# patrikhuber/superviseddescent

Hardware: AMD Instinct MI355X
Metric: faces/sec RCR-22 detect (batch 4096) (higher is better)
Workload: dtype f32; 1 GPU; RCR-22 detect, batch 4096 synthetic 256x256 u8 faces per GPU, 4 cascade levels (UoCTTI HOG 5x5 cells, cell 11/10/8/6, 4 orientations, F=8801, M=44), model trained on-GPU on 100000 synthetic faces (shipped .bin absent from the reference checkout); batch_per_gpu=4096, levels=4

## Files before the change

### superviseddescent_amd/csrc/sdm_apply.hip

```cpp
#include "sdm_kernels.h"
#include <stdlib.h>

#pragma clang fp contract(off)
#include "sdm_ied.h"

namespace {

typedef float f32x4 __attribute__((ext_vector_type(4)));

#define APPLY_WAVES 4

template <int RT, int NT>
__global__ void __launch_bounds__(APPLY_WAVES * 64)
apply_partial_kernel(const float* __restrict__ feat, long long ldf, int N, int kgroups,
                     const float* __restrict__ Rt, long long ldr, float* __restrict__ partial, int splits)
{
    __shared__ float red[APPLY_WAVES - 1][RT * NT][4][64];
    const int lane = threadIdx.x & 63, wave = threadIdx.x >> 6;
    const int li = lane & 15, lq = lane >> 4;
    const int row0 = blockIdx.x * (16 * RT);
    const int split = blockIdx.y;
    const int g0 = (int)(((long long)kgroups * split) / splits);
    const int g1 = (int)(((long long)kgroups * (split + 1)) / splits);

// ... 265 lines not shown
    for (int o = 32; o; o >>= 1) v = __builtin_fmaxf(v, __shfl_xor(v, o));
    if ((threadIdx.x & 63) == 0) part[threadIdx.x >> 6] = v;
    __syncthreads();
    if (threadIdx.x == 0) out[blockIdx.x] = __builtin_bit_cast(unsigned, __builtin_fmaxf(__builtin_fmaxf(part[0], part[1]), __builtin_fmaxf(part[2], part[3])));
}

__global__ void __launch_bounds__(256) apply_planes_kernel(const float* __restrict__ Rt, long long ldr, int Mp, int KG, af16x8* __restrict__ planes,
                                                           const unsigned* __restrict__ rmax)
{
    const long long u = (long long)blockIdx.x * 256 + threadIdx.x;
    if (u >= (long long)KG * Mp) return;
    const int kg = (int)(u / Mp), col = (int)(u % Mp);
    const float scale = __builtin_ldexpf(1.0f, 14 - apply_f16_exponent(rmax[col]));
    const float* src = Rt + (long long)col * ldr + 8 * kg;
    af16x8 p1, p2;
#pragma unroll
    for (int j = 0; j < 8; ++j) {
        const float v = src[j] * scale;
        const _Float16 h1 = (_Float16)v;
        p1[j] = h1; p2[j] = (_Float16)(v - (float)h1);
    }
    planes[u] = p1; planes[(size_t)KG * Mp + u] = p2;
}

__global__ void apply_reduce_kernel(const float* __restrict__ partial, int splits, int N, int Mp, int M,
                                    const float* __restrict__ x_in, float* __restrict__ x_out, int L,
                                    EyeIdxDev eyes)
{
    const long long t = (long long)blockIdx.x * blockDim.x + threadIdx.x;
    if (t >= (long long)N * M) return;
    const int row = (int)(t / M), col = (int)(t - (long long)row * M);
    const float* xr = x_in + (long long)row * M;
    const float xc = xr[col];
    float scale = 1.0f;
    if (eyes.nre > 0) {
        const float n = (float)(1.0 / device_ied_rows(xr, L, eyes));
        scale = 1.0f / n;
    }
    float u = 0.0f;
    const float* pp = partial + (long long)row * Mp + col;
    const long long sstride = (long long)N * Mp;
    constexpr int RB = 24;
    for (int s0 = 0; s0 < splits; s0 += RB) {
        float v[RB];
#pragma unroll
        for (int j = 0; j < RB; ++j) v[j] = pp[(long long)(s0 + j < splits ? s0 + j : splits - 1) * sstride];
#pragma unroll
        for (int j = 0; j < RB; ++j) u = s0 + j < splits ? u + v[j] : u;
    }
    x_out[t] = xc - u * scale;
}

__global__ void targets_kernel(const float* __restrict__ x, const float* __restrict__ xstar, int N, int L,
                               EyeIdxDev eyes, float* __restrict__ feat, long long ldf, int bcol0)
{
    const int M = 2 * L;
    const long long t = (long long)blockIdx.x * blockDim.x + threadIdx.x;
    if (t >= (long long)N * M) return;
    const int row = (int)(t / M), col = (int)(t - (long long)row * M);
    const float* xr = x + (long long)row * M;
    float n = 1.0f;
    if (eyes.nre > 0) n = (float)(1.0 / device_ied_rows(xr, L, eyes));
    feat[(long long)row * ldf + bcol0 + col] = (xr[col] - xstar[t]) * n;
}

__global__ void pack_regressor_kernel(const float* __restrict__ Rsol, int F, int M, int Mp, float* __restrict__ Rt,
                                      long long ldf, float* __restrict__ Rc)
{
    const long long t = (long long)blockIdx.x * blockDim.x + threadIdx.x;
    if (t >= (long long)Mp * ldf) return;
    const int j = (int)(t / ldf);
    const long long k = t - (long long)j * ldf;
    const float v = (k < F && j < M) ? Rsol[k * Mp + j] : 0.0f;
    Rt[t] = v;
    if (Rc && k < F && j < M) Rc[k * M + j] = v;
}

__global__ void subtract_templates_kernel(float* __restrict__ feat, long long ldf, const float* __restrict__ tmpl, int N, int F)
{
    const long long t = (long long)blockIdx.x * blockDim.x + threadIdx.x;
    if (t >= (long long)N * F) return;
    const int row = (int)(t / F), col = (int)(t - (long long)row * F);
    feat[(long long)row * ldf + col] -= tmpl[t];
// ... 251 lines not shown
```

### superviseddescent_amd/csrc/sdm_capi_context.hip

```cpp
#include "sdm_capi_internal.h"

extern "C" {

const char* sdm_last_error(void) { return err_string().c_str(); }

int sdm_device_count(void)
{
    int n = 0;
    if (hipGetDeviceCount(&n) != hipSuccess) return 0;
    return n;
}

sdm_ctx* sdm_create(int device)
{
    int n = 0;
    if (hipGetDeviceCount(&n) != hipSuccess || n <= 0) {
        fail(SDM_ERR_NO_DEVICE, "no HIP device available: this engine has no CPU fallback");
        return nullptr;
    }
    if (device < 0 || device >= n) { fail(SDM_ERR_INVALID, "device index out of range"); return nullptr; }
    hipDeviceProp_t prop;
    if (hipGetDeviceProperties(&prop, device) != hipSuccess) { fail(SDM_ERR_HIP, "hipGetDeviceProperties failed"); return nullptr; }
    if (strncmp(prop.gcnArchName, "gfx950", 6) != 0) {
        fail(SDM_ERR_NO_DEVICE, std::string("device is ") + prop.gcnArchName + ", kernels are built for gfx950 only");
// ... 7 lines not shown
    }
    c->own_stream = true;
    int prio_least = 0, prio_greatest = 0;
    (void)hipDeviceGetStreamPriorityRange(&prio_least, &prio_greatest);
    if (hipStreamCreateWithPriority(&c->solve_aux.stream, hipStreamNonBlocking, prio_least) != hipSuccess ||
        hipEventCreateWithFlags(&c->solve_aux.chain_done, hipEventDisableTiming) != hipSuccess ||
        hipEventCreateWithFlags(&c->solve_aux.tail_done, hipEventDisableTiming) != hipSuccess) {
        fail(SDM_ERR_HIP, "hipStreamCreate failed"); delete c; return nullptr;
    }
    if (c->status.ensure(1, true, c->stream) || c->lambda_dev.ensure(1, true, c->stream)) { delete c; return nullptr; }
    for (int b = 0; b < sdm_ctx::XBLOCKS_MAX; ++b)
        if (hipEventCreateWithFlags(&c->gram_ev[b], hipEventDisableTiming) != hipSuccess) { fail(SDM_ERR_HIP, "hipEventCreate failed"); delete c; return nullptr; }
    if (hipEventCreateWithFlags(&c->gram_xdone, hipEventDisableTiming) != hipSuccess) { fail(SDM_ERR_HIP, "hipEventCreate failed"); delete c; return nullptr; }
    return c;
}

void sdm_destroy(sdm_ctx* c)
{
    if (!c) return;
    hipError_t e = hipSetDevice(c->device); (void)e;
    e = hipStreamSynchronize(c->stream);
    if (c->solve_aux.stream) {
        e = hipStreamSynchronize(c->solve_aux.stream);
        e = hipEventDestroy(c->solve_aux.chain_done); e = hipEventDestroy(c->solve_aux.tail_done);
        for (int b = 0; b < sdm_ctx::XBLOCKS_MAX; ++b) if (c->gram_ev[b]) e = hipEventDestroy(c->gram_ev[b]);
        if (c->gram_xdone) e = hipEventDestroy(c->gram_xdone);
        e = hipStreamDestroy(c->solve_aux.stream);
    }
    drain_timing(c);
    for (auto ev : c->pool) { e = hipEventDestroy(ev); }
    c->img_owned.release(); c->img_off.release(); c->img_w.release(); c->img_h.release();
    c->img_stride.release(); c->img_idx.release(); c->x[0].release(); c->x[1].release();
    c->xstar.release(); c->tmpl.release(); c->feat.release(); c->patch_idx.release(); c->status.release();
    c->partial.release(); c->shard_stage.release(); c->G.release(); c->gpack.release(); c->fro.release(); c->Rsol.release(); c->winv.release(); c->gram_planes.release(); c->gram_flag.release(); c->upd_planes.release(); c->upd_maxdiag.release(); c->lambda_dev.release();
    for (auto& r : c->Rp) r.release();
    for (auto& r : c->Rd) r.release();
    c->cells.release(); c->qr_work.release();
    c->Rmax.release();
    c->pose.release();
    c->track.release();
    c->align.release();
    c->sweep.release();
    c->frames.release();
    c->upright.release();
    c->warp.release();
    for (auto& r : c->Rt) r.release();
    for (auto& q : c->plans) { q.lane_tab.release(); q.wb.release(); q.wb16.release(); q.pass_info.release(); q.cut.release(); q.taps.release(); q.pair_taps.release(); }
    if (c->own_stream) e = hipStreamDestroy(c->stream);
    delete c;
}

int sdm_set_stream(sdm_ctx* c, void* hip_stream)
{
    if (!c) return fail(SDM_ERR_INVALID, "null context");
    HIP_TRY(hipStreamSynchronize(c->stream));
    if (c->own_stream) { HIP_TRY(hipStreamDestroy(c->stream)); c->own_stream = false; }
    c->stream = (hipStream_t)hip_stream;
    return SDM_OK;
}

int sdm_synchronize(sdm_ctx* c)
{
    if (!c) return fail(SDM_ERR_INVALID, "null context");
    HIP_TRY(hipStreamSynchronize(c->stream));
    drain_timing(c);
    return SDM_OK;
}
// ... 393 lines not shown
```

### superviseddescent_amd/csrc/sdm_capi_debug.hip

```cpp
#include "sdm_capi_internal.h"

extern "C" {

int sdm_gram_device_ptr(sdm_ctx* c, void** p, size_t* count)
{
    if (!c || c->g_level < 0) return fail(SDM_ERR_INVALID, "no Gram matrix");
    *p = c->G.p; *count = (size_t)c->g_fp * c->g_ncols;
    return SDM_OK;
}

int sdm_x_device_ptr(sdm_ctx* c, void** p, size_t* count)
{
    if (!c || c->N <= 0) return fail(SDM_ERR_INVALID, "no x");
    *p = c->x[c->cur].p; *count = (size_t)c->N * c->M;
    return SDM_OK;
}

int sdm_features_device_ptr(sdm_ctx* c, void** p, long long* ld, int* n_rows)
{
    if (!c || c->feat_level < 0) return fail(SDM_ERR_INVALID, "no features");
    *p = c->feat.p; *ld = c->ldf; *n_rows = c->N;
    c->feat_bounded = false;
    return SDM_OK;
}
// ... 172 lines not shown
    if (!c) return fail(SDM_ERR_INVALID, "null context");
    c->fuse_apply = fused != 0;
    c->fuse_wide = fused == 2;
    c->split_store = split_store != 0;
    return SDM_OK;
}

int sdm_debug_gradient_table(sdm_ctx* c, int level, float* g, int* bin)
{
    if (!c || level < 0 || level >= (int)c->levels.size() || !g || !bin) return fail(SDM_ERR_INVALID, "bad arguments");
    HIP_TRY(hipSetDevice(c->device));
    const size_t n = 511 * 511;
    ScopedBuf<float> d_g; ScopedBuf<int> d_b;
    int rc;
    if ((rc = d_g.ensure(n)) || (rc = d_b.ensure(n))) return rc;
    sdm_launch_gradient_table(c->levels[level], d_g.p, d_b.p, c->stream);
    HIP_TRY(hipGetLastError());
    HIP_TRY(hipMemcpyAsync(g, d_g.p, n * sizeof(float), hipMemcpyDeviceToHost, c->stream));
    HIP_TRY(hipMemcpyAsync(bin, d_b.p, n * sizeof(int), hipMemcpyDeviceToHost, c->stream));
    HIP_TRY(hipStreamSynchronize(c->stream));
    d_g.release(); d_b.release();
    return SDM_OK;
}

int sdm_debug_set_option(sdm_ctx* c, const char* name, int value)
{
    if (!c || !name) return fail(SDM_ERR_INVALID, "bad arguments");
    const std::string n(name);
    if (n == "hog_no_pack") c->packing = value == 0;
    else if (n == "hog_two_load") c->hog_two_load = value != 0;
    else if (n == "hog_split_store") c->split_store = value != 0;
    else if (n == "detect_unfused") c->fuse_apply = value == 0;
    else if (n == "detect_fuse_wide") c->env_fuse_wide = value != 0;
    else if (n == "apply_f32") c->env_apply_f32 = value != 0;
    else if (n == "gram_f32") c->env_gram_f32 = value != 0;
    else if (n == "gram_bf16x3") c->env_gram_bf16 = value != 0;
    else if (n == "update_f32") c->solve_aux.upd_f32_only = value != 0 ? 1 : 0;
    else if (n == "gram_xblocks") c->env_xblocks = value;
    else if (n == "solve_upd_min_tiles") c->solve_aux.upd_min_tiles = value;
    else if (n == "solve_fine_head") c->solve_aux.fine_head_max = value;
    else if (n == "solve_bs_cap") c->solve_aux.bs_cap = value;
    else if (n == "solve_shard_emulate") c->env_shard_emulate = value;
    else return fail(SDM_ERR_INVALID, "sdm_debug_set_option: unknown option " + n);
    return SDM_OK;
}

int sdm_debug_update_f16(sdm_ctx* c, const float* P_host, int rows, int wcols, int wcols_factor, float factor_bound, float* C_host)
{
    if (!c || !P_host || !C_host || rows <= 0 || rows > 512 || rows % 128 || wcols <= 0 || wcols % 128 || wcols_factor <= 0 || wcols_factor > wcols || wcols_factor % 128)
        return fail(SDM_ERR_INVALID, "bad arguments");
    HIP_TRY(hipSetDevice(c->device));
    ScopedBuf<float> dP, dC; ScopedBuf<unsigned char> planes; ScopedBuf<unsigned> scales; ScopedBuf<int> status;
    int rc;
    if ((rc = dP.ensure((size_t)rows * wcols)) || (rc = dC.ensure((size_t)wcols * wcols)) || (rc = planes.ensure(sdm_update_f16_plane_bytes(512, wcols))) ||
        (rc = scales.ensure(4)) || (rc = status.ensure(1, true, c->stream)))
        return rc;
    HIP_TRY(hipMemcpyAsync(dP.p, P_host, (size_t)rows * wcols * sizeof(float), hipMemcpyHostToDevice, c->stream));
    HIP_TRY(hipMemcpyAsync(dC.p, C_host, (size_t)wcols * wcols * sizeof(float), hipMemcpyHostToDevice, c->stream));
    const unsigned sc[4] = {__builtin_bit_cast(unsigned, factor_bound), 0u, 0u, __builtin_bit_cast(unsigned, factor_bound)};
    HIP_TRY(hipMemcpyAsync(scales.p, sc, sizeof(sc), hipMemcpyHostToDevice, c->stream));
    sdm_launch_update_split_f16(dP.p, wcols, rows, wcols, wcols_factor, planes.p, scales.p, 0, status.p, c->stream, false);
    sdm_launch_update_f16(planes.p, rows, wcols, wcols_factor, dC.p, wcols, scales.p, 0, 0, 1 << 30, 0, 1, c->stream, 0);
    HIP_TRY(hipGetLastError());
    int st = 0;
    HIP_TRY(hipMemcpyAsync(&st, status.p, sizeof(int), hipMemcpyDeviceToHost, c->stream));
    HIP_TRY(hipMemcpyAsync(C_host, dC.p, (size_t)wcols * wcols * sizeof(float), hipMemcpyDeviceToHost, c->stream));
// ... 7 lines not shown
```

### superviseddescent_amd/csrc/sdm_capi_detect.hip

```cpp
#include "sdm_capi_internal.h"

namespace sdm_capi {

void fill_row_tab(HogLevelDev& lv)
{
    for (int d = 0; d < 64 && d < lv.S; ++d) {
        const HogRowConst rc = packed_row_const(d, lv.cell, lv.C);
        lv.row_tab[d][0] = rc.ws0;
        lv.row_tab[d][1] = rc.ws1;
        memcpy(&lv.row_tab[d][2], &rc.band, sizeof(int));
        lv.row_tab[d][3] = rc.w2;
    }
}



void drain_timing(sdm_ctx* c)
{
    for (auto& p : c->pending) {
        hipError_t e = hipEventSynchronize(p.b); (void)e;
        float ms = 0.f;
        if (hipEventElapsedTime(&ms, p.a, p.b) == hipSuccess) { c->t_ms[p.slot] += ms; c->t_n[p.slot] += 1; }
        if (!p.a_shared) c->pool.push_back(p.a);
        c->pool.push_back(p.b);
// ... 157 lines not shown
{
    if (c->feat_level != level) return fail(SDM_ERR_INVALID, "sdm_apply: features of this level not extracted");
    if (!c->have_R[level]) return fail(SDM_ERR_INVALID, "sdm_apply: no regressor set for this level");
    const int F = level_F(c, level);
    const int splits = sdm_apply_splits(c->N, F, c->M);
    int rc = c->partial.ensure((size_t)splits * c->N * Mp_of(c->M));
    if (rc) return rc;
    {
        Timer t(c, SDM_T_APPLY);
        sdm_launch_apply(c->feat.p, c->ldf, c->N, F, c->Rt[level].p, c->ldf, c->M, c->x[c->cur].p,
                         c->x[c->cur ^ 1].p, c->L, c->eyes, c->partial.p, splits, c->stream,
                         (c->feat_bounded && !c->env_apply_f32) ? c->Rp[level].p : nullptr,
                         (c->feat_bounded && !c->env_apply_f32 && c->Rp[level].p) ? c->Rmax.p + (size_t)level * Mp_of(c->M) : nullptr);
    }
    HIP_TRY(hipGetLastError());
    c->cur ^= 1;
    return SDM_OK;
}

bool fused_ok(const sdm_ctx* c, int level)
{
    return c->fuse_apply && (Mp_of(c->M) <= 64 || c->env_fuse_wide || c->fuse_wide) && split_ok(c, level) && c->have_R[level] && c->Rd[level].p &&
           c->Rp[level].p && c->tmpl_N == 0;
}
int detect_level_fused(sdm_ctx* c, int l)
{
    { const int rci = hog_checks(c, l); if (rci) return rci; }
    const int Mp = Mp_of(c->M);
    int rc;
    size_t cells_max = 0;
    for (size_t q = 0; q < c->levels.size(); ++q) { const size_t n = sdm_cells_floats(c->levels[q], c->N, c->L); if (n > cells_max) cells_max = n; }
    if ((rc = c->cells.ensure(cells_max)) || (rc = c->partial.ensure((size_t)c->L * c->N * Mp))) return rc;
    const HogLevelDev& lv = c->levels[l];
    {
        Timer t(c, SDM_T_HOG);
        sdm_launch_hog_cells(image_set(c), sample_index(c), c->x[c->cur].p, c->N, c->L, c->eyes, lv,
                             cells_plan(c, l), c->cells.p, c->patch_idx.p, c->status.p, c->stream);
    }
    {
        Timer t(c, SDM_T_APPLY);
        sdm_launch_desc_apply(lv, c->cells.p, c->plans[l].cut.p, c->N, c->L, c->M, c->Rd[l].p, c->Rmax.p + (size_t)l * Mp,
                              c->Rt[l].p, c->ldf, c->partial.p, c->stream);
        sdm_launch_apply_reduce(c->partial.p, c->L, c->N, c->M, c->x[c->cur].p, c->x[c->cur ^ 1].p, c->L, c->eyes, c->stream);
    }
    HIP_TRY(hipGetLastError());
    c->cur ^= 1;
    c->feat_level = -1;
    c->have_patch_idx = true;
    return SDM_OK;
}

int detect_level(sdm_ctx* c, int l)
{
    if (fused_ok(c, l)) return detect_level_fused(c, l);
    int rc = do_hog(c, l);
    if (!rc) rc = do_apply(c, l);
    return rc;
}

}

extern "C" {

int sdm_hog_features(sdm_ctx* c, int level, float* feat_host)
{
    if (!c || level < 0 || level >= (int)c->levels.size()) return fail(SDM_ERR_INVALID, "bad level");
    HIP_TRY(hipSetDevice(c->device));
    int rc = do_hog(c, level);
    if (rc) return rc;
    if (feat_host) {
        const int F = level_F(c, level);
        HIP_TRY(hipMemcpy2DAsync(feat_host, (size_t)F * sizeof(float), c->feat.p, (size_t)c->ldf * sizeof(float),
                                 (size_t)F * sizeof(float), c->N, hipMemcpyDeviceToHost, c->stream));
        HIP_TRY(hipStreamSynchronize(c->stream));
        return check_status(c);
    }
// ... 70 lines not shown
```

### superviseddescent_amd/csrc/sdm_capi_internal.h

```cpp
#pragma once
#include "../../include/sdm.h"
#include "sdm_kernels.h"

#include <dlfcn.h>
#include <limits.h>
#include <math.h>
#include <stdio.h>
#include <stdlib.h>
#include <string.h>
#include <string>
#include <vector>

namespace sdm_capi {


inline std::string& err_string() { static thread_local std::string e; return e; }

inline int fail(int code, const std::string& msg)
{
    err_string() = msg;
    return code;
}

constexpr long long SDM_FUSED_MAX_STRIDE = 1ll << 20;
// ... 77 lines not shown
    bool env_gram_f32 = false;
    bool env_gram_bf16 = false;
    int env_shard_emulate = 0;
    int hog_mode = SDM_HOG_COLUMNS;
    int Fmax = 0;
    long long ldf = 0;
    int rhs_tiles = 1;

    DevBuf<uint8_t> img_owned;
    const uint8_t* img_base = nullptr;
    DevBuf<long long> img_off;
    DevBuf<int> img_w, img_h, img_stride;
    int n_images = 0;
    bool narrow_images = false;
    DevBuf<int> img_idx;
    bool idx_identity = true;
    int n_idx = 0, max_idx = -1;

    int N = 0;
    DevBuf<float> x[2];
    int cur = 0;
    DevBuf<float> xstar;
    DevBuf<float> tmpl;
    int tmpl_F = 0, tmpl_N = 0;
    bool have_targets = false;
    DevBuf<float> feat;
    int feat_level = -1;
    int feat_wide_F = 0, feat_wide_N = 0;
    bool feat_bounded = false;
    DevBuf<int> patch_idx;
    bool have_patch_idx = false;
    DevBuf<int> status;
    DevBuf<float> partial;

    std::vector<DevBuf<float>> Rt;
    std::vector<DevBuf<unsigned char>> Rp;
    std::vector<DevBuf<unsigned char>> Rd;
    DevBuf<unsigned> Rmax;
    std::vector<bool> have_R;

    DevBuf<float> G;
    DevBuf<float> gpack;
    int g_ncols = 0;
    int g_fp = 0;
    int g_level = -1;
    DevBuf<double> fro;
    DevBuf<float> Rsol;
    DevBuf<float> winv;
    DevBuf<int> gram_flag;
    static const int XBLOCKS_MAX = 8;
    hipEvent_t gram_ev[XBLOCKS_MAX] = {}; hipEvent_t gram_xdone = nullptr;
    int gram_blocks = 0;
    int gram_block_c[XBLOCKS_MAX + 1] = {};
    int env_xblocks = -1;
    int gram_fallbacks = 0;
    int update_range_fallbacks = 0;
    int gram_f32_fallbacks = 0;
    DevBuf<unsigned char> gram_planes;
    DevBuf<float> lambda_dev;

    sdm_allreduce_fn allreduce = nullptr;
    void* allreduce_user = nullptr;
    int world_size = 1;
    void* rccl_comm = nullptr;
    int (*rccl_allreduce)(const void*, void*, size_t, int, int, void*, hipStream_t) = nullptr;
    int shard_rank = 0, shard_world = 0;
// ... 214 lines not shown
```

### superviseddescent_amd/csrc/sdm_desc.hip

```cpp
#include "sdm_kernels.h"
#include <stdlib.h>

#pragma clang fp contract(off)

namespace {

typedef float f32x4 __attribute__((ext_vector_type(4)));
typedef _Float16 f16x8 __attribute__((ext_vector_type(8)));
typedef unsigned u32x4 __attribute__((ext_vector_type(4)));

#define DS_WAVES 8
#ifndef DS_MINW
#define DS_MINW 6
#endif
#ifndef DS_ABL
#define DS_ABL 0
#endif

__host__ __device__ constexpr int desc_dim(int O, int variant) { return variant == 1 ? 3 * O + 4 : 4 * O; }
__host__ __device__ constexpr int desc_dp(int D) { return (D + 7) / 8 * 8; }
__host__ __device__ constexpr int desc_pk(int CC, int D) { return CC * desc_dp(D); }
__host__ __device__ constexpr int desc_kp(int P) { return (P + 31) / 32 * 32; }
__host__ __device__ constexpr int desc_ks(int P) { return ((P + 7) / 8) * 8 + 8; }
__host__ __device__ constexpr size_t desc_stage_bytes(int P, int FB) { return (size_t)2 * FB * desc_ks(P) * 2 + 64; }

__device__ inline int desc_f16_exponent(unsigned maxbits)
{
    const float b = __builtin_bit_cast(float, maxbits);
    if (!(b > 0.0f) || !(b < 3.0e38f)) return 14;
    return (int)((maxbits >> 23) & 0xff) - 127;
}

__host__ __device__ constexpr int desc_kparts(int PK) { return desc_kp(PK) / 32 <= 14 ? 2 : 4; }
__host__ __device__ constexpr int desc_nw(int PK, int W) { return W / desc_kparts(PK); }

template <int TO, int TC, int VARIANT, bool FUSED, int FB, int W = DS_WAVES, bool ONE = false>
__global__ void __launch_bounds__(W * 64, (TO > 4 && !FUSED) ? 2 : ((TO <= 4 && FUSED) ? DS_MINW : 4))
desc_kernel(const float* __restrict__ cells, const int* __restrict__ cut, int N, int L,
            float* __restrict__ feat, long long ldf, int has_bias,
            const u32x4* __restrict__ planes, int NT, const unsigned* __restrict__ rmax, const float* __restrict__ Rt, long long ldr,
            float* __restrict__ partial)
{
    constexpr int O = TO, C = TC, CC = C * C, D = desc_dim(TO, VARIANT), P = CC * D;
    constexpr int DP = desc_dp(D), PK = desc_pk(CC, D);
    constexpr int KP = desc_kp(PK), KS = desc_ks(PK), KSTEPS = KP / 32, MT = FB / 16;
    static_assert(CC <= 32, "one cell per lane, two patches per wave");
    extern __shared__ __attribute__((aligned(16))) unsigned char smem[];
    unsigned short* stage_hi = (unsigned short*)smem;
    unsigned short* stage_lo = stage_hi + (size_t)FB * KS;
    const int lane = threadIdx.x & 63, wave = threadIdx.x >> 6;
    const int tile = blockIdx.x / L, l = blockIdx.x - tile * L;
    const int half = lane >> 5, cell = lane & 31;
    const bool active = cell < CC;
    const int cc = active ? cell : CC - 1;
    const int x = cc / C, y = cc - x * C, ct = x * C + y, ci = y * C + x;
    const int xm = x > 0 ? x - 1 : 0, xp = x < C - 1 ? x + 1 : C - 1, ym = y > 0 ? y - 1 : 0, yp = y < C - 1 ? y + 1 : C - 1;
    const int lb = half * 32;
    const int iA = (lb + xm * C + ym) * 4, iB = (lb + x * C + ym) * 4, iC = (lb + xp * C + ym) * 4;
    const int iD = (lb + xm * C + y) * 4, iF = (lb + xp * C + y) * 4;
    const int iG = (lb + xm * C + yp) * 4, iH = (lb + x * C + yp) * 4, iI = (lb + xp * C + yp) * 4;
    const unsigned ipk0 = iA | iB << 8 | iC << 16 | iD << 24, ipk1 = iF | iG << 8 | iH << 16 | iI << 24;
    const int cutw = cut[l];
    const bool is_cut = (cutw & 1) != 0;
    const bool ld0 = x <= ((cutw >> 8) & 0xff), ld1 = x >= ((cutw >> 16) & 0xff);

    if (FUSED) {
        constexpr int PADW = KS - PK;
        for (int i = threadIdx.x; i < 2 * FB * PADW; i += W * 64) {
            const int piece = i / (FB * PADW), r = i - piece * (FB * PADW);
            const int m = r / PADW, k = PK + (r - m * PADW);
            (piece ? stage_lo : stage_hi)[(size_t)m * KS + k] = 0;
        }
        if (threadIdx.x < 32) ((unsigned short*)smem)[(size_t)2 * FB * KS + threadIdx.x] = 0;
    }

// ... 210 lines not shown
        }
    }
    }
    __syncthreads();
    float* red = (float*)smem;
    if (kp > 0) {
#pragma unroll
        for (int ti = 0; ti < MAXT; ++ti) {
            const int nt = ntl + ti * NW;
            if (nt >= NT) continue;
#pragma unroll
            for (int mt = 0; mt < MT; ++mt)
#pragma unroll
                for (int e = 0; e < 4; ++e) red[((((size_t)(kp - 1) * NT + nt) * MT + mt) * 4 + e) * 64 + lane_p] = acc[ti][mt][e];
        }
    }
    __syncthreads();
    if (kp == 0) {
#pragma unroll
        for (int ti = 0; ti < MAXT; ++ti) {
            const int nt = ntl + ti * NW;
            if (nt >= NT) continue;
            const int col = 16 * nt + li;
            const float unscale = __builtin_ldexpf(1.0f, -12 + (desc_f16_exponent(rmx[ti]) - 14));
            const float bias = biasv[ti];
#pragma unroll
            for (int mt = 0; mt < MT; ++mt)
#pragma unroll
                for (int e = 0; e < 4; ++e) {
                    float v = acc[ti][mt][e];
#pragma unroll
                    for (int q = 1; q < KPARTS; ++q) v += red[((((size_t)(q - 1) * NT + nt) * MT + mt) * 4 + e) * 64 + lane_p];
                    const int face = tile * FB + 16 * mt + 4 * lq + e;
                    if (face < N) partial[((long long)l * N + face) * Mp + col] = v * unscale + bias;
                }
        }
    }
}

__global__ void __launch_bounds__(256) desc_planes_kernel(const float* __restrict__ Rt, long long ldr, int L, int P, int C, int D, int DP, int KSTEPS, int NT,
                                                          const unsigned* __restrict__ rmax, f16x8* __restrict__ planes)
{
    const long long u = (long long)blockIdx.x * 256 + threadIdx.x;
    if (u >= (long long)L * KSTEPS * NT * 64) return;
    const int lane = (int)(u & 63);
    const long long frag = u >> 6;
    const int nt = (int)(frag % NT), ks = (int)((frag / NT) % KSTEPS), l = (int)(frag / ((long long)NT * KSTEPS));
    const int col = 16 * nt + (lane & 15), k0 = 32 * ks + 8 * (lane >> 4);
    const float scale = __builtin_ldexpf(1.0f, 14 - desc_f16_exponent(rmax[col]));
    const float* src = Rt + (long long)col * ldr + (long long)l * P;
    const int CC = C * C;
    f16x8 p1, p2;
#pragma unroll
    for (int j = 0; j < 8; ++j) {
        const int kk = k0 + j, cell = kk / DP, f = kk - cell * DP;
        const int y = cell / C, x = cell - y * C, ct = x * C + y;
        const float v = (cell < CC && f < D) ? src[f * CC + ct] * scale : 0.0f;
        const _Float16 h1 = (_Float16)v;
        p1[j] = h1; p2[j] = (_Float16)(v - (float)h1);
    }
    planes[frag * 128 + lane] = p1;
    planes[frag * 128 + 64 + lane] = p2;
}

template <int TO, int VARIANT, bool FUSED, int FB, int W = DS_WAVES, bool ONE = false>
void launch_desc(const float* cells, const int* cut, int N, int L, float* feat, long long ldf, int has_bias, const void* planes, int NT,
                 const unsigned* rmax, const float* Rt, long long ldr, float* partial, hipStream_t stream)
{
    const size_t lds = FUSED ? desc_stage_bytes(desc_pk(25, desc_dim(TO, VARIANT)), FB) + (FB == 16 ? 40 * 1024 : 0) : 0;
    const unsigned grid = (unsigned)(((long long)N + FB - 1) / FB * L);
    static unsigned long long seen = 0;
    if (FUSED && sdm_first_use_on_device(seen))
        SDM_SET_ATTR((const void*)desc_kernel<TO, 5, VARIANT, FUSED, FB, W, ONE>, hipFuncAttributeMaxDynamicSharedMemorySize, 160 * 1024);
    hipLaunchKernelGGL((desc_kernel<TO, 5, VARIANT, FUSED, FB, W, ONE>), dim3(grid), dim3(W * 64), lds, stream, cells, cut, N, L, feat, ldf,
                       has_bias, (const u32x4*)planes, NT, rmax, Rt, ldr, partial);
}

}

bool sdm_desc_supported(const HogLevelDev& lv) { return lv.C == 5 && (lv.O == 4 || lv.O == 9) && (lv.variant == 0 || lv.variant == 1); }

size_t sdm_cells_floats(const HogLevelDev& lv, int N, int L) { return (size_t)N * L * 2 * 2 * lv.O * lv.C * lv.C + 4; }

void sdm_launch_desc_store(const HogLevelDev& lv, const float* cells, const int* cut, int N, int L, float* feat, long long ldf, hipStream_t stream)
{
    if (N <= 0) return;
    const int hb = lv.fixed_h == 0 ? 1 : 0;
#define DS(O, V) launch_desc<O, V, false, 64>(cells, cut, N, L, feat, ldf, hb, nullptr, 0, nullptr, nullptr, 0, nullptr, stream)
    if (lv.O == 4) { if (lv.variant == 1) DS(4, 1); else DS(4, 0); }
    else { if (lv.variant == 1) DS(9, 1); else DS(9, 0); }
#undef DS
}

size_t sdm_desc_planes_bytes(const HogLevelDev& lv, int L, int M)
{
    const int KSTEPS = desc_kp(desc_pk(lv.C * lv.C, desc_dim(lv.O, lv.variant))) / 32, NT = (M + 15) / 16;
    return ((size_t)L * KSTEPS + 1) * NT * 2 * 64 * 16;
}

void sdm_launch_desc_planes(const HogLevelDev& lv, const float* Rt, long long ldr, int L, int M, const unsigned* rmax, void* planes, hipStream_t stream)
{
    const int D = desc_dim(lv.O, lv.variant), DP = desc_dp(D);
    const int KSTEPS = desc_kp(desc_pk(lv.C * lv.C, D)) / 32, NT = (M + 15) / 16;
    const long long total = (long long)L * KSTEPS * NT * 64;
    hipLaunchKernelGGL(desc_planes_kernel, dim3((unsigned)((total + 255) / 256)), dim3(256), 0, stream, Rt, ldr, L, lv.P, lv.C, D, DP, KSTEPS, NT, rmax, (f16x8*)planes);
    hipError_t e = hipMemsetAsync((unsigned char*)planes + (size_t)L * KSTEPS * NT * 2 * 64 * 16, 0, (size_t)NT * 2 * 64 * 16, stream); (void)e;
}

void sdm_launch_desc_apply(const HogLevelDev& lv, const float* cells, const int* cut, int N, int L, int M, const void* planes,
                           const unsigned* rmax, const float* Rt, long long ldr, float* partial, hipStream_t stream)
{
    if (N <= 0) return;
    const int hb = lv.fixed_h == 0 ? 1 : 0, NT = (M + 15) / 16;
#define DA(O, V, FB) do { \
        if (NT <= desc_nw(desc_pk(25, desc_dim(O, V)), DS_WAVES)) launch_desc<O, V, true, FB, DS_WAVES, true>(cells, cut, N, L, nullptr, 0, hb, planes, NT, rmax, Rt, ldr, partial, stream); \
        else launch_desc<O, V, true, FB>(cells, cut, N, L, nullptr, 0, hb, planes, NT, rmax, Rt, ldr, partial, stream); \
    } while (0)
    if (lv.O == 4) { if (lv.variant == 1) DA(4, 1, 32); else DA(4, 0, 32); }
    else { if (lv.variant == 1) DA(9, 1, 16); else DA(9, 0, 16); }
#undef DA
}
```

### superviseddescent_amd/csrc/sdm_ied.h

```cpp
#pragma once
#include "sdm_kernels.h"

__device__ inline double device_ied_rows(const float* __restrict__ xr, int L, const EyeIdxDev& e)
{
    float rx = 0.0f, ry = 0.0f, lx = 0.0f, ly = 0.0f;
    float vrx[SDM_MAX_EYE], vry[SDM_MAX_EYE], vlx[SDM_MAX_EYE], vly[SDM_MAX_EYE];
#pragma unroll
    for (int i = 0; i < SDM_MAX_EYE; ++i) {
        const int ir = e.re[i < e.nre ? i : 0], il = e.le[i < e.nle ? i : 0];
        vrx[i] = xr[ir]; vry[i] = xr[ir + L]; vlx[i] = xr[il]; vly[i] = xr[il + L];
    }
#pragma unroll
    for (int i = 0; i < SDM_MAX_EYE; ++i) {
        if (i < e.nre) { rx += vrx[i]; ry += vry[i]; }
        if (i < e.nle) { lx += vlx[i]; ly += vly[i]; }
    }
    rx /= (float)e.nre; ry /= (float)e.nre;
    lx /= (float)e.nle; ly /= (float)e.nle;
    float dxf = rx - lx, dyf = ry - ly;
    double dx = dxf, dy = dyf;
    return sqrt(dx * dx + dy * dy);
}
```

### superviseddescent_amd/csrc/sdm_kernels.h

```cpp
#pragma once
#include <hip/hip_runtime.h>
#include <cstdio>
#include <stdint.h>
#include "sdm_align_tensor_device.h"

#define SDM_SCALE_TAB 128
#define SDM_MAX_ORIENT 16
#define SDM_MAX_EYE 4

struct HogLevelDev {
    int variant;
    int C;
    int cell;
    int O;
    int S;
    int D;
    int P;
    float rel;
    int fixed_h;
    float ox[SDM_MAX_ORIENT];
    float oy[SDM_MAX_ORIENT];
    int n_sector;
    float sector_t[SDM_MAX_ORIENT / 2];
    alignas(16) float row_tab[64][4];
// ... 62 lines not shown
template <int CELL, int C>
struct HogRowConstTable {
    HogRowConst r[C * CELL] = {};
    constexpr HogRowConstTable() { for (int d = 0; d < C * CELL; ++d) r[d] = packed_row_const(d, CELL, C); }
};
const HogRowConst* sdm_hog_compiled_row_consts(int cell, int C);
#ifdef __cplusplus
#include <vector>
struct HogPlanHost {
    int G = 0, P = 0, n_main = 0, Gt = 0, Pt = 0, hist_slots = 2;
    std::vector<unsigned> lane_tab;
    std::vector<float> wb;
    std::vector<unsigned short> wb16;
    std::vector<int> pass_info;
    std::vector<int> cut;
};
bool sdm_hog_plan_build(const HogLevelDev& lv, int L, HogPlanHost& out);
#endif
void sdm_launch_hog_packed(const ImageSetDev& imgs, const int* img_idx, const float* x, int N, int L,
                           const EyeIdxDev& eyes, const HogLevelDev& lv, const HogPlanDev& plan, float* feat, long long ldf,
                           int* idx_out, int* status, hipStream_t stream);

void sdm_launch_hog_cells(const ImageSetDev& imgs, const int* img_idx, const float* x, int N, int L,
                          const EyeIdxDev& eyes, const HogLevelDev& lv, const HogPlanDev& plan, float* cells,
                          int* idx_out, int* status, hipStream_t stream);
bool sdm_hog_cells_row_carry(const HogLevelDev& lv, const HogPlanDev& plan);
bool sdm_hog_cells_pair_carry(const HogLevelDev& lv, const HogPlanDev& plan);

bool sdm_desc_supported(const HogLevelDev& lv);
size_t sdm_cells_floats(const HogLevelDev& lv, int N, int L);
void sdm_launch_desc_store(const HogLevelDev& lv, const float* cells, const int* cut, int N, int L, float* feat, long long ldf, hipStream_t stream);
size_t sdm_desc_planes_bytes(const HogLevelDev& lv, int L, int M);
void sdm_launch_desc_planes(const HogLevelDev& lv, const float* Rt, long long ldr, int L, int M, const unsigned* rmax, void* planes, hipStream_t stream);
void sdm_launch_desc_apply(const HogLevelDev& lv, const float* cells, const int* cut, int N, int L, int M, const void* planes,
                           const unsigned* rmax, const float* Rt, long long ldr, float* partial, hipStream_t stream);
void sdm_launch_apply_reduce(const float* partial, int splits, int N, int M, const float* x_in, float* x_out, int L,
                             const EyeIdxDev& eyes, hipStream_t stream);

size_t sdm_colpiv_qr_work_floats(int F);
bool sdm_colpiv_qr_supported(int F);
void sdm_launch_colpiv_qr_solve(float* G, long long ldg, int F, int rhs0, int nrhs, float* R_out, long long ldr, int r_rows,
                                float* work, int** rank_dev_out, hipStream_t stream);

void sdm_launch_hog_fast_profile(const ImageSetDev& imgs, const int* img_idx, const float* x, int N, int L,
                                 const EyeIdxDev& eyes, const HogLevelDev& lv, float* feat, long long ldf,
                                 int* status, unsigned long long* prof_dev, hipStream_t stream);

void sdm_launch_hog_debug(const ImageSetDev& imgs, const int* img_idx, const float* x, int N, int L,
                          const EyeIdxDev& eyes, const HogLevelDev& lv, int sample, int landmark,
                          uint8_t* rsz_out, uint8_t* bins_out, float* hist_out, float* desc_out,
                          int* status, hipStream_t stream);

void sdm_launch_gradient_table(const HogLevelDev& lv, float* g_out, int* bin_out, hipStream_t stream);

int sdm_apply_splits(int N, int F, int M);
void sdm_launch_apply(const float* feat, long long ldf, int N, int F, const float* Rt, long long ldr,
                      int M, const float* x_in, float* x_out, int L, const EyeIdxDev& eyes,
                      float* partial, int splits, hipStream_t stream, const void* planes = nullptr, const unsigned* rmax = nullptr);
size_t sdm_apply_planes_bytes(long long ldr, int M);
void sdm_launch_apply_planes(const float* Rt, long long ldr, int M, void* planes, unsigned* rmax, hipStream_t stream);

void sdm_launch_pack_regressor(const float* Rsol, int F, int M, int Mp, float* Rt, long long ldf, float* Rc, hipStream_t stream);
void sdm_launch_subtract_templates(float* feat, long long ldf, const float* tmpl, int N, int F, hipStream_t stream);

void sdm_launch_bgr2gray(const uint8_t* bgr, uint8_t* gray, long long n_pixels, int shift, hipStream_t stream);

struct FrameConvDev {
    const uint8_t* src;
// ... 185 lines not shown
```

### superviseddescent_amd/engine.py

```python
from __future__ import annotations

import ctypes
import os
from dataclasses import dataclass
from typing import Callable, List, Optional, Sequence

import numpy as np

from . import _lib, ibug
from ._lib import SdmError, SdmHogParam, check


@dataclass
class HoGParam:

    vlhog_variant: int
    num_cells: int
    cell_size: int
    num_bins: int
    relative_patch_size: float

    @property
    def dim(self) -> int:
        return 3 * self.num_bins + 4 if self.vlhog_variant == 1 else 4 * self.num_bins

    @property
    def patch_dim(self) -> int:
        return self.num_cells * self.num_cells * self.dim


def _device_frames(images) -> bool:
    if getattr(images, "is_cuda", False):
        return True
    if isinstance(images, (list, tuple)) and len(images):
        return bool(getattr(images[0], "is_cuda", False)) or isinstance(images[0], tuple)
    return False


def _fp(a: np.ndarray):
    return a.ctypes.data_as(ctypes.POINTER(ctypes.c_float))


def _ip(a: np.ndarray):
    return a.ctypes.data_as(ctypes.POINTER(ctypes.c_int))


_DEV_OPTIONS = ("hog_no_pack", "hog_two_load", "hog_split_store", "detect_unfused", "detect_fuse_wide", "apply_f32", "gram_f32", "gram_bf16x3", "update_f32",
                "gram_xblocks", "solve_upd_min_tiles", "solve_fine_head", "solve_bs_cap", "solve_shard_emulate")


class Context:

    def __init__(self, device: int = 0, stream: Optional[int] = None):
        self._lib = _lib.lib()
        self._h = self._lib.sdm_create(int(device))
        if not self._h:
            raise SdmError(_lib.SDM_ERR_NO_DEVICE, self._lib.sdm_last_error().decode())
        self.device = device
        self._keep = []
        for key, val in os.environ.items():
            if key.startswith("SDM_") and key[4:].lower() in _DEV_OPTIONS:
                self.set_option(key[4:].lower(), int(val))
        if stream is not None:
            check(self._lib.sdm_set_stream(self._h, ctypes.c_void_p(stream)))
        self.L = 0
        self.n_levels = 0
        self.align_channels = 1
        self._resident = {}

    def set_option(self, name: str, value: int):
        check(self._lib.sdm_debug_set_option(self._h, name.encode(), int(value)))

    def close(self):
        if getattr(self, "_h", None):
            self._lib.sdm_destroy(self._h)
            self._h = None

    def __del__(self):
        try:
            self.close()
# ... 1797 lines not shown
```

Measured before the change: 4.424 million faces/s.

## Fuse apply-reduce update into descriptor apply kernel via last-block tickets

The fused descriptor-apply kernel now does the shape update itself. Each block publishes its per-landmark partials, then increments a per-tile atomic ticket. The last block to arrive for a tile sums the partials across landmarks and writes the updated shapes. This removes the separate apply_reduce launch and its partial reread latency per cascade level. The cost is release/acquire fences, atomic stores and loads, and a tail of serial reduction work in one block per tile. A ticket buffer must stay zeroed between launches.

```diff
diff --git a/superviseddescent_amd/csrc/sdm_apply.hip b/superviseddescent_amd/csrc/sdm_apply.hip
--- a/superviseddescent_amd/csrc/sdm_apply.hip
+++ b/superviseddescent_amd/csrc/sdm_apply.hip
@@ -321,11 +321,7 @@
     const int row = (int)(t / M), col = (int)(t - (long long)row * M);
     const float* xr = x_in + (long long)row * M;
     const float xc = xr[col];
-    float scale = 1.0f;
-    if (eyes.nre > 0) {
-        const float n = (float)(1.0 / device_ied_rows(xr, L, eyes));
-        scale = 1.0f / n;
-    }
+    const float scale = device_update_scale(xr, L, eyes);
     float u = 0.0f;
     const float* pp = partial + (long long)row * Mp + col;
     const long long sstride = (long long)N * Mp;
@@ -337,7 +333,7 @@
 #pragma unroll
         for (int j = 0; j < RB; ++j) u = s0 + j < splits ? u + v[j] : u;
     }
-    x_out[t] = xc - u * scale;
+    x_out[t] = device_update(xc, u, scale);
 }
 
 __global__ void targets_kernel(const float* __restrict__ x, const float* __restrict__ xstar, int N, int L,
diff --git a/superviseddescent_amd/csrc/sdm_capi_context.hip b/superviseddescent_amd/csrc/sdm_capi_context.hip
--- a/superviseddescent_amd/csrc/sdm_capi_context.hip
+++ b/superviseddescent_amd/csrc/sdm_capi_context.hip
@@ -63,7 +63,7 @@
     c->img_owned.release(); c->img_off.release(); c->img_w.release(); c->img_h.release();
     c->img_stride.release(); c->img_idx.release(); c->x[0].release(); c->x[1].release();
     c->xstar.release(); c->tmpl.release(); c->feat.release(); c->patch_idx.release(); c->status.release();
-    c->partial.release(); c->shard_stage.release(); c->G.release(); c->gpack.release(); c->fro.release(); c->Rsol.release(); c->winv.release(); c->gram_planes.release(); c->gram_flag.release(); c->upd_planes.release(); c->upd_maxdiag.release(); c->lambda_dev.release();
+    c->partial.release(); c->tickets.release(); c->shard_stage.release(); c->G.release(); c->gpack.release(); c->fro.release(); c->Rsol.release(); c->winv.release(); c->gram_planes.release(); c->gram_flag.release(); c->upd_planes.release(); c->upd_maxdiag.release(); c->lambda_dev.release();
     for (auto& r : c->Rp) r.release();
     for (auto& r : c->Rd) r.release();
     c->cells.release(); c->qr_work.release();
diff --git a/superviseddescent_amd/csrc/sdm_capi_debug.hip b/superviseddescent_amd/csrc/sdm_capi_debug.hip
--- a/superviseddescent_amd/csrc/sdm_capi_debug.hip
+++ b/superviseddescent_amd/csrc/sdm_capi_debug.hip
@@ -228,6 +228,7 @@
     else if (n == "hog_split_store") c->split_store = value != 0;
     else if (n == "detect_unfused") c->fuse_apply = value == 0;
     else if (n == "detect_fuse_wide") c->env_fuse_wide = value != 0;
+    else if (n == "detect_separate_update") c->separate_update = value != 0;
     else if (n == "apply_f32") c->env_apply_f32 = value != 0;
     else if (n == "gram_f32") c->env_gram_f32 = value != 0;
     else if (n == "gram_bf16x3") c->env_gram_bf16 = value != 0;
diff --git a/superviseddescent_amd/csrc/sdm_capi_detect.hip b/superviseddescent_amd/csrc/sdm_capi_detect.hip
--- a/superviseddescent_amd/csrc/sdm_capi_detect.hip
+++ b/superviseddescent_amd/csrc/sdm_capi_detect.hip
@@ -213,6 +213,8 @@
     for (size_t q = 0; q < c->levels.size(); ++q) { const size_t n = sdm_cells_floats(c->levels[q], c->N, c->L); if (n > cells_max) cells_max = n; }
     if ((rc = c->cells.ensure(cells_max)) || (rc = c->partial.ensure((size_t)c->L * c->N * Mp))) return rc;
     const HogLevelDev& lv = c->levels[l];
+    const bool in_launch = !c->separate_update && sdm_desc_apply_updates(lv, c->M);
+    if (in_launch && (rc = c->tickets.ensure(sdm_desc_tickets(c->N), true, c->stream))) return rc;
     {
         Timer t(c, SDM_T_HOG);
         sdm_launch_hog_cells(image_set(c), sample_index(c), c->x[c->cur].p, c->N, c->L, c->eyes, lv,
@@ -220,9 +222,10 @@
     }
     {
         Timer t(c, SDM_T_APPLY);
-        sdm_launch_desc_apply(lv, c->cells.p, c->plans[l].cut.p, c->N, c->L, c->M, c->Rd[l].p, c->Rmax.p + (size_t)l * Mp,
-                              c->Rt[l].p, c->ldf, c->partial.p, c->stream);
-        sdm_launch_apply_reduce(c->partial.p, c->L, c->N, c->M, c->x[c->cur].p, c->x[c->cur ^ 1].p, c->L, c->eyes, c->stream);
+        const bool updated = sdm_launch_desc_apply(lv, c->cells.p, c->plans[l].cut.p, c->N, c->L, c->M, c->Rd[l].p, c->Rmax.p + (size_t)l * Mp,
+                                                   c->Rt[l].p, c->ldf, c->partial.p, c->stream, c->x[c->cur].p, c->x[c->cur ^ 1].p, &c->eyes,
+                                                   in_launch ? c->tickets.p : nullptr);
+        if (!updated) sdm_launch_apply_reduce(c->partial.p, c->L, c->N, c->M, c->x[c->cur].p, c->x[c->cur ^ 1].p, c->L, c->eyes, c->stream);
     }
     HIP_TRY(hipGetLastError());
     c->cur ^= 1;
diff --git a/superviseddescent_amd/csrc/sdm_capi_internal.h b/superviseddescent_amd/csrc/sdm_capi_internal.h
--- a/superviseddescent_amd/csrc/sdm_capi_internal.h
+++ b/superviseddescent_amd/csrc/sdm_capi_internal.h
@@ -133,6 +133,8 @@
     bool have_patch_idx = false;
     DevBuf<int> status;
     DevBuf<float> partial;
+    DevBuf<int> tickets;
+    bool separate_update = false;
 
     std::vector<DevBuf<float>> Rt;
     std::vector<DevBuf<unsigned char>> Rp;
diff --git a/superviseddescent_amd/csrc/sdm_desc.hip b/superviseddescent_amd/csrc/sdm_desc.hip
--- a/superviseddescent_amd/csrc/sdm_desc.hip
+++ b/superviseddescent_amd/csrc/sdm_desc.hip
@@ -1,4 +1,5 @@
 #include "sdm_kernels.h"
+#include "sdm_ied.h"
 #include <stdlib.h>
 
 #pragma clang fp contract(off)
@@ -16,6 +17,9 @@
 #ifndef DS_ABL
 #define DS_ABL 0
 #endif
+#ifndef DS_PUBLISH
+#define DS_PUBLISH 3
+#endif
 
 __host__ __device__ constexpr int desc_dim(int O, int variant) { return variant == 1 ? 3 * O + 4 : 4 * O; }
 __host__ __device__ constexpr int desc_dp(int D) { return (D + 7) / 8 * 8; }
@@ -34,13 +38,15 @@
 __host__ __device__ constexpr int desc_kparts(int PK) { return desc_kp(PK) / 32 <= 14 ? 2 : 4; }
 __host__ __device__ constexpr int desc_nw(int PK, int W) { return W / desc_kparts(PK); }
 
-template <int TO, int TC, int VARIANT, bool FUSED, int FB, int W = DS_WAVES, bool ONE = false>
+template <int TO, int TC, int VARIANT, bool FUSED, int FB, int W = DS_WAVES, bool ONE = false, bool UPD = false>
 __global__ void __launch_bounds__(W * 64, (TO > 4 && !FUSED) ? 2 : ((TO <= 4 && FUSED) ? DS_MINW : 4))
 desc_kernel(const float* __restrict__ cells, const int* __restrict__ cut, int N, int L,
             float* __restrict__ feat, long long ldf, int has_bias,
             const u32x4* __restrict__ planes, int NT, const unsigned* __restrict__ rmax, const float* __restrict__ Rt, long long ldr,
-            float* __restrict__ partial)
-{
+            float* __restrict__ partial,
+            const float* __restrict__ x_in, float* __restrict__ x_out, EyeIdxDev eyes, int M, int* __restrict__ tickets)
+{
+    static_assert(!UPD || (FUSED && ONE), "the update is the one-tile-per-wave fused instance's");
     constexpr int O = TO, C = TC, CC = C * C, D = desc_dim(TO, VARIANT), P = CC * D;
     constexpr int DP = desc_dp(D), PK = desc_pk(CC, D);
     constexpr int KP = desc_kp(PK), KS = desc_ks(PK), KSTEPS = KP / 32, MT = FB / 16;
@@ -317,8 +323,51 @@
 #pragma unroll
                     for (int q = 1; q < KPARTS; ++q) v += red[((((size_t)(q - 1) * NT + nt) * MT + mt) * 4 + e) * 64 + lane_p];
                     const int face = tile * FB + 16 * mt + 4 * lq + e;
+                    if constexpr (UPD && DS_PUBLISH != 1) {
+                        if (face < N) __hip_atomic_store(partial + ((long long)l * N + face) * Mp + col, v * unscale + bias, __ATOMIC_RELAXED, __HIP_MEMORY_SCOPE_AGENT);
+                    } else
                     if (face < N) partial[((long long)l * N + face) * Mp + col] = v * unscale + bias;
                 }
+        }
+    }
+    if constexpr (UPD) {
+        if (kp == 0 && ntl < NT) {
+            if (DS_PUBLISH == 2) __builtin_amdgcn_fence(__ATOMIC_RELEASE, "agent");
+            asm volatile("s_waitcnt vmcnt(0)" ::: "memory");
+        }
+        __syncthreads();
+        int* drawn = (int*)smem;
+        if (tx == 0) {
+            if (DS_PUBLISH < 2) __builtin_amdgcn_fence(__ATOMIC_RELEASE, "agent");
+            asm volatile("s_waitcnt vmcnt(0)" ::: "memory");
+            drawn[0] = __hip_atomic_fetch_add(tickets + tile, 1, __ATOMIC_RELAXED, __HIP_MEMORY_SCOPE_AGENT);
+        }
+        __syncthreads();
+        if (drawn[0] != L - 1) return;
+        if (tx == 0) __hip_atomic_store(tickets + tile, 0, __ATOMIC_RELAXED, __HIP_MEMORY_SCOPE_AGENT);
+        __builtin_amdgcn_fence(__ATOMIC_ACQUIRE, "agent");
+        asm volatile("s_waitcnt vmcnt(0)" ::: "memory");
+        const float* xt = x_in + (long long)tile * FB * M;
+        float* xo = x_out + (long long)tile * FB * M;
+        const float* pt = partial + (long long)tile * FB * Mp;
+        const long long sstride = (long long)N * Mp;
+        constexpr int RB = 24;
+        for (int o = (int)tx; o < nf * M; o += W * 64) {
+            const int row = o / M, col = o - row * M;
+            const float* xr = xt + row * M;
+            const float xc = xr[col];
+            const float scale = device_update_scale(xr, L, eyes);
+            const float* pp = pt + row * Mp + col;
+            float u = 0.0f;
+            for (int s0 = 0; s0 < L; s0 += RB) {
+                float pv[RB];
+#pragma unroll
+                for (int j = 0; j < RB; ++j) pv[j] = __hip_atomic_load(pp + (long long)(s0 + j < L ? s0 + j : L - 1) * sstride, __ATOMIC_RELAXED, __HIP_MEMORY_SCOPE_AGENT);
+                __builtin_amdgcn_sched_barrier(0);
+#pragma unroll
+                for (int j = 0; j < RB; ++j) u = s0 + j < L ? u + pv[j] : u;
+            }
+            xo[o] = device_update(xc, u, scale);
         }
     }
 }
@@ -348,17 +397,19 @@
     planes[frag * 128 + 64 + lane] = p2;
 }
 
-template <int TO, int VARIANT, bool FUSED, int FB, int W = DS_WAVES, bool ONE = false>
+struct DescUpdate { const float* x_in; float* x_out; EyeIdxDev eyes; int M; int* tickets; };
+
+template <int TO, int VARIANT, bool FUSED, int FB, int W = DS_WAVES, bool ONE = false, bool UPD = false>
 void launch_desc(const float* cells, const int* cut, int N, int L, float* feat, long long ldf, int has_bias, const void* planes, int NT,
-                 const unsigned* rmax, const float* Rt, long long ldr, float* partial, hipStream_t stream)
+                 const unsigned* rmax, const float* Rt, long long ldr, float* partial, hipStream_t stream, const DescUpdate& up = DescUpdate{})
 {
     const size_t lds = FUSED ? desc_stage_bytes(desc_pk(25, desc_dim(TO, VARIANT)), FB) + (FB == 16 ? 40 * 1024 : 0) : 0;
     const unsigned grid = (unsigned)(((long long)N + FB - 1) / FB * L);
     static unsigned long long seen = 0;
     if (FUSED && sdm_first_use_on_device(seen))
-        SDM_SET_ATTR((const void*)desc_kernel<TO, 5, VARIANT, FUSED, FB, W, ONE>, hipFuncAttributeMaxDynamicSharedMemorySize, 160 * 1024);
-    hipLaunchKernelGGL((desc_kernel<TO, 5, VARIANT, FUSED, FB, W, ONE>), dim3(grid), dim3(W * 64), lds, stream, cells, cut, N, L, feat, ldf,
-                       has_bias, (const u32x4*)planes, NT, rmax, Rt, ldr, partial);
+        SDM_SET_ATTR((const void*)desc_kernel<TO, 5, VARIANT, FUSED, FB, W, ONE, UPD>, hipFuncAttributeMaxDynamicSharedMemorySize, 160 * 1024);
+    hipLaunchKernelGGL((desc_kernel<TO, 5, VARIANT, FUSED, FB, W, ONE, UPD>), dim3(grid), dim3(W * 64), lds, stream, cells, cut, N, L, feat, ldf,
+                       has_bias, (const u32x4*)planes, NT, rmax, Rt, ldr, partial, up.x_in, up.x_out, up.eyes, up.M, up.tickets);
 }
 
 }
@@ -392,16 +443,28 @@
     hipError_t e = hipMemsetAsync((unsigned char*)planes + (size_t)L * KSTEPS * NT * 2 * 64 * 16, 0, (size_t)NT * 2 * 64 * 16, stream); (void)e;
 }
 
-void sdm_launch_desc_apply(const HogLevelDev& lv, const float* cells, const int* cut, int N, int L, int M, const void* planes,
-                           const unsigned* rmax, const float* Rt, long long ldr, float* partial, hipStream_t stream)
-{
-    if (N <= 0) return;
+bool sdm_desc_apply_updates(const HogLevelDev& lv, int M)
+{
+    return lv.O == 4 && (M + 15) / 16 <= desc_nw(desc_pk(25, desc_dim(4, lv.variant)), DS_WAVES);
+}
+size_t sdm_desc_tickets(int N) { return ((size_t)N + 31) / 32; }
+
+bool sdm_launch_desc_apply(const HogLevelDev& lv, const float* cells, const int* cut, int N, int L, int M, const void* planes,
+                           const unsigned* rmax, const float* Rt, long long ldr, float* partial, hipStream_t stream,
+                           const float* x_in, float* x_out, const EyeIdxDev* eyes, int* tickets)
+{
+    if (N <= 0) return false;
     const int hb = lv.fixed_h == 0 ? 1 : 0, NT = (M + 15) / 16;
+    const bool upd = tickets && x_in && x_out && eyes && sdm_desc_apply_updates(lv, M);
 #define DA(O, V, FB) do { \
         if (NT <= desc_nw(desc_pk(25, desc_dim(O, V)), DS_WAVES)) launch_desc<O, V, true, FB, DS_WAVES, true>(cells, cut, N, L, nullptr, 0, hb, planes, NT, rmax, Rt, ldr, partial, stream); \
         else launch_desc<O, V, true, FB>(cells, cut, N, L, nullptr, 0, hb, planes, NT, rmax, Rt, ldr, partial, stream); \
     } while (0)
-    if (lv.O == 4) { if (lv.variant == 1) DA(4, 1, 32); else DA(4, 0, 32); }
+#define DU(V) launch_desc<4, V, true, 32, DS_WAVES, true, true>(cells, cut, N, L, nullptr, 0, hb, planes, NT, rmax, Rt, ldr, partial, stream, DescUpdate{x_in, x_out, *eyes, M, tickets})
+    if (upd) { if (lv.variant == 1) DU(1); else DU(0); }
+    else if (lv.O == 4) { if (lv.variant == 1) DA(4, 1, 32); else DA(4, 0, 32); }
     else { if (lv.variant == 1) DA(9, 1, 16); else DA(9, 0, 16); }
+#undef DU
 #undef DA
-}
+    return upd;
+}
diff --git a/superviseddescent_amd/csrc/sdm_ied.h b/superviseddescent_amd/csrc/sdm_ied.h
--- a/superviseddescent_amd/csrc/sdm_ied.h
+++ b/superviseddescent_amd/csrc/sdm_ied.h
@@ -21,3 +21,17 @@
     double dx = dxf, dy = dyf;
     return sqrt(dx * dx + dy * dy);
 }
+
+#if defined(__clang__)
+#pragma clang fp contract(off)
+#endif
+__device__ inline float device_update_scale(const float* __restrict__ xr, int L, const EyeIdxDev& eyes)
+{
+    float scale = 1.0f;
+    if (eyes.nre > 0) {
+        const float n = (float)(1.0 / device_ied_rows(xr, L, eyes));
+        scale = 1.0f / n;
+    }
+    return scale;
+}
+__device__ inline float device_update(float xc, float u, float scale) { return xc - u * scale; }
diff --git a/superviseddescent_amd/csrc/sdm_kernels.h b/superviseddescent_amd/csrc/sdm_kernels.h
--- a/superviseddescent_amd/csrc/sdm_kernels.h
+++ b/superviseddescent_amd/csrc/sdm_kernels.h
@@ -118,8 +118,11 @@
 void sdm_launch_desc_store(const HogLevelDev& lv, const float* cells, const int* cut, int N, int L, float* feat, long long ldf, hipStream_t stream);
 size_t sdm_desc_planes_bytes(const HogLevelDev& lv, int L, int M);
 void sdm_launch_desc_planes(const HogLevelDev& lv, const float* Rt, long long ldr, int L, int M, const unsigned* rmax, void* planes, hipStream_t stream);
-void sdm_launch_desc_apply(const HogLevelDev& lv, const float* cells, const int* cut, int N, int L, int M, const void* planes,
-                           const unsigned* rmax, const float* Rt, long long ldr, float* partial, hipStream_t stream);
+bool sdm_desc_apply_updates(const HogLevelDev& lv, int M);
+size_t sdm_desc_tickets(int N);
+bool sdm_launch_desc_apply(const HogLevelDev& lv, const float* cells, const int* cut, int N, int L, int M, const void* planes,
+                           const unsigned* rmax, const float* Rt, long long ldr, float* partial, hipStream_t stream,
+                           const float* x_in = nullptr, float* x_out = nullptr, const EyeIdxDev* eyes = nullptr, int* tickets = nullptr);
 void sdm_launch_apply_reduce(const float* partial, int splits, int N, int M, const float* x_in, float* x_out, int L,
                              const EyeIdxDev& eyes, hipStream_t stream);
 
diff --git a/superviseddescent_amd/engine.py b/superviseddescent_amd/engine.py
--- a/superviseddescent_amd/engine.py
+++ b/superviseddescent_amd/engine.py
@@ -45,7 +45,7 @@
     return a.ctypes.data_as(ctypes.POINTER(ctypes.c_int))
 
 
-_DEV_OPTIONS = ("hog_no_pack", "hog_two_load", "hog_split_store", "detect_unfused", "detect_fuse_wide", "apply_f32", "gram_f32", "gram_bf16x3", "update_f32",
+_DEV_OPTIONS = ("hog_no_pack", "hog_two_load", "hog_split_store", "detect_unfused", "detect_fuse_wide", "detect_separate_update", "apply_f32", "gram_f32", "gram_bf16x3", "update_f32",
                 "gram_xblocks", "solve_upd_min_tiles", "solve_fine_head", "solve_bs_cap", "solve_shard_emulate")
 
 
```

Result: slower. 3.728 million faces/s (-15.7%).
